# AI4quantum/twisteRL

Hardware: NVIDIA B200
Metric: rollout env-steps/sec incl. policy fwd (puzzle15 PPO) (higher is better)
Workload: dtype f16f8c (tcgen05; main products one-hot x table and h1 x W in fp16, their two correction products (table residue, activation residue) as fp8 MMAs, f32 accumulate; same 1e-3 bar as f16x2w16, tests/test_gpu_precision.py)

## Files before the change

### twisterl_b200/csrc/twr_forward_tc2.cu

```cuda
#include "twr_kernels.cuh"
#include "twr_tc_ptx.cuh"
#include "twr_step.cuh"

#include <atomic>
#include <cstdlib>
#include <cuda.h>
#include <cuda_fp16.h>
#include <cuda_fp8.h>
#include <map>
#include <mutex>

extern std::atomic<long long> g_twr_launches;

namespace {

constexpr int TM = 128;
constexpr int NTHREADS = 320;
constexpr int NEPI = 256;
constexpr int TILE_BYTES = 16384;
constexpr int NSLOTS = 8;
constexpr int MAX_KB1 = 4;
constexpr int MAX_OBS = 32;
constexpr int NCOPIES = 1;

constexpr int SM_A1 = 0;
constexpr int SM_RING = SM_A1 + MAX_KB1 * TILE_BYTES;
constexpr int SM_A8 = SM_RING;
constexpr int A8_TILES = 2;
constexpr int SM_MISC = SM_RING + NSLOTS * TILE_BYTES;
constexpr int SM_HEADW = SM_MISC;
constexpr int SM_B1 = SM_HEADW + 8192;
constexpr int SM_EMBB = SM_B1 + 1024;
constexpr int SM_PART = SM_EMBB + 4096;
constexpr int SM_PERM = SM_PART + 2 * TM * 8 * 4;
constexpr int SM_OPERM = SM_PERM + 4 * TM;
constexpr int OPERM_MAX = 2048;
constexpr int SM_BARS = SM_OPERM + OPERM_MAX;
constexpr int SM_TOTAL = SM_BARS + 512;
static_assert(SM_TOTAL <= 227 * 1024, "shared memory budget");

enum Bar { B_FULL0 = 0, B_EMPTY0 = NSLOTS, B_A1_FULL = 2 * NSLOTS, B_A1_EMPTY, B_D1_FULL0, B_D1_FULL1,
// ... 264 lines not shown
    float* headw = reinterpret_cast<float*>(smem + SM_HEADW);
    float* b1s = reinterpret_cast<float*>(smem + SM_B1);
    float* embb = reinterpret_cast<float*>(smem + SM_EMBB);
    float* part_s = reinterpret_cast<float*>(smem + SM_PART);
    int8_t* perm_s = reinterpret_cast<int8_t*>(smem + SM_PERM);
    uint8_t* operm_s = smem + SM_OPERM;
    const bool operm_smem = p.n_perms > 0 && p.obs_size <= 256 && p.n_perms * p.obs_size <= OPERM_MAX;
    const int NC = t.NC, NKB1 = t.NKB1;
    constexpr int H = HT;
    constexpr bool F8 = TERMS >= 16;
    static_assert(!F8 || TERMS == 19, "fp8 corrections replace exactly the terms of f16x2w16");
    constexpr int NS = F8 ? NSLOTS - A8_TILES : NSLOTS;
    constexpr int RING = F8 ? SM_RING + A8_TILES * TILE_BYTES : SM_RING;
    const int terms = TERMS >= 0 ? (TERMS & 7) : (a.tc_terms ? (a.tc_terms & 7) : 7);
    const bool g1_lo = (terms & 1) != 0, g2_alo = (terms & 2) != 0, g2_wlo = (terms & 4) != 0;
    const int NKB8 = t.NKB8;
    constexpr uint32_t idesc2 = H == 256 ? IDESC_256x256 : IDESC_256x128;
    constexpr int g2_units = H == 256 ? 4 : 2;

    if (threadIdx.x == 0) {
        for (int i = 0; i < NSLOTS; ++i) { mbar_init(bar(B_FULL0 + i), 1); mbar_init(bar(B_EMPTY0 + i), 1); }
        mbar_init(bar(B_A1_FULL), 2 * TM); mbar_init(bar(B_A1_EMPTY), 1);
        mbar_init(bar(B_D1_FULL0), 1); mbar_init(bar(B_D1_FULL1), 1);
        mbar_init(bar(B_A2_FULL0), 2 * NEPI); mbar_init(bar(B_A2_FULL1), 2 * NEPI);
        mbar_init(bar(B_D2_FULL), 1); mbar_init(bar(B_D2_EMPTY), 2 * NEPI);
        asm volatile("fence.mbarrier_init.release.cluster;" ::: "memory");
    }
    for (int i = threadIdx.x; i < (MAX_KB1 + (F8 ? A8_TILES : 0)) * TILE_BYTES / 16; i += NTHREADS)
        reinterpret_cast<uint4*>(smem + SM_A1)[i] = make_uint4(0, 0, 0, 0);
    for (int i = threadIdx.x; i < H; i += NTHREADS) {
        for (int o = 0; o < 4; ++o) headw[o * H + i] = o < p.A ? p.wa[(size_t)i * p.A + o] : 0.0f;
        headw[4 * H + i] = p.wv[i];
        b1s[i] = p.b1[i];
    }
    for (int i = threadIdx.x; i < t.E; i += NTHREADS) embb[i] = F8 ? p.emb_b[i] * H1_SCALE8 : p.emb_b[i];
    if (operm_smem)
        for (int i = threadIdx.x; i < p.n_perms * p.obs_size; i += NTHREADS) operm_s[i] = (uint8_t)p.obs_perms[i];
    uint8_t* aperm_s = smem + SM_BARS + 384;
    const bool aperm_smem = p.n_perms > 0 && p.n_perms * p.A <= 128;
    if (aperm_smem)
        for (int i = threadIdx.x; i < p.n_perms * p.A; i += NTHREADS) aperm_s[i] = (uint8_t)p.act_perms[i];
    if (warp == 1) {
        asm volatile("tcgen05.alloc.cta_group::2.sync.aligned.shared::cta.b32 [%0], %1;" ::"r"(smem_u32(tmem_slot)), "r"(512u));
        asm volatile("tcgen05.relinquish_alloc_permit.cta_group::2.sync.aligned;");
    }
    fence_async_smem();
    tc_fence_before();
    __syncthreads();
    cluster_sync();
    tc_fence_after();
    const uint32_t tmem = *tmem_slot;
    const uint32_t D2_COL = 0, D1_COL = 256;
    const bool timed = a.dbg != nullptr;
    long long* trace = (timed && blockIdx.x == 0) ? a.dbg + 148 * 16 : nullptr;
    auto stamp = [&](int item, int ev) { if (trace && item < 8) trace[item * 32 + ev] = clock64(); };

    if (warp == 0) {
        if (lane == 0) {
            const int img_row0 = t.row0 + ((pair_id % NCOPIES) * 2 + crank) * (int)slots_per_rank(t) * (TILE_BYTES / 128);
            const int g1_row0 = img_row0, g2_row0 = img_row0 + (int)slots_g1(t) * (TILE_BYTES / 128);
            uint32_t use = 0;
            long long w_empty = 0;
            auto push = [&](int row) {
                const uint32_t slot = use % NS, round = use / NS;
                mbar_wait_t(bar(B_EMPTY0 + slot), (round & 1u) ^ 1u, w_empty, timed);
                if (a.dbg_flags & 2) {
                    if (crank == 0) mbar_arrive(bar(B_FULL0 + slot));
                } else {
                    if (crank == 0) mbar_expect_tx(bar(B_FULL0 + slot), 2 * TILE_BYTES);
                    tma_load_2sm(sbase + RING + slot * TILE_BYTES, &tmap, 0, row, bar(B_FULL0 + slot));
                }
                ++use;
            };
            auto push_g1 = [&](int sc) {
                for (int i = 0; i < 2 * NKB1; ++i)
                    if (!(i & 1) || g1_lo) push(g1_row0 + (sc * 2 * NKB1 + i) * (TILE_BYTES / 128));
            };
            auto push_g2 = [&](int j) {
                for (int u = 0; u < g2_units; ++u)
                    if (!(u & 1) || g2_wlo) push(g2_row0 + (j * g2_units + u) * (TILE_BYTES / 128));
            };
            if constexpr (F8) {
                const int n1 = NKB1 + NKB8, n2 = 2 * (H == 256 ? 3 : 2);
                for (int it = 0; it < n_items; ++it)
                    for (int sc = 0; sc < NC / 2; ++sc) {
                        for (int u = 0; u < n1; ++u) push(g1_row0 + (sc * n1 + u) * (TILE_BYTES / 128));
                        for (int u = 0; u < n2; ++u) push(g2_row0 + (sc * n2 + u) * (TILE_BYTES / 128));
                    }
            } else {
                for (int it = 0; it < n_items; ++it)
                    for (int sc = 0; sc < NC / 2; ++sc) { push_g1(sc); push_g2(2 * sc); push_g2(2 * sc + 1); }
            }
            if (a.dbg) a.dbg[blockIdx.x * 16 + 8] = w_empty;
        }
        __syncwarp();
    } else if (warp == 1) {
        if (lane == 0 && crank == 0) {
            uint32_t use = 0, d1use = 0, a2use = 0;
            long long w_slot = 0, w_a1 = 0, w_a2 = 0, w_d2 = 0, w_slot_g1 = 0, w_slot_first = 0;
            const long long t_begin = clock64();
            auto wait_slot = [&]() -> uint32_t {
                const uint32_t slot = use % NS, round = use / NS;
                mbar_wait_cluster_t(bar(B_FULL0 + slot), round & 1u, w_slot, timed);
                tc_fence_after();
                ++use;
                return slot;
            };
            for (int it = 0; it < n_items; ++it) {
                mbar_wait_cluster_t(bar(B_A1_FULL), it & 1, w_a1, timed);
                tc_fence_after();
                stamp(it, 0);
                auto g1 = [&](int sc) {
                    stamp(it, 1 + 2 * sc);
                    const uint32_t d = tmem + D1_COL;
                    if constexpr (F8) {
                        constexpr uint32_t I8_256 = idesc8(256, 1, 0), I8_128 = idesc8(128, 1, 0);
                        const bool on = !(a.dbg_flags & 8);
                        for (int kb = 0; kb < NKB1 - 1; ++kb) {
                            const uint64_t ad = make_desc(sbase + SM_A1 + kb * TILE_BYTES);
// ... 158 lines not shown
                                const uint32_t sidx = H == 256 ? (uint32_t)((u >> 1) * 4 + ks) : (uint32_t)ks;
                                const uint32_t ah = a_base + 32u * (sidx >> 1) + 8u * (sidx & 1u);
                                const uint64_t bk = H == 256 ? bd + 2u * ks : bd + (uint64_t)((ks >> 2) * (8192 >> 4)) + 2u * (ks & 3);
                                tc2_mma_ts(d, ah, bk, idesc2, !(first && ks == 0));
                                if (part == 0 && g2_alo) tc2_mma_ts(d, ah + 16u, bk, idesc2, 1u);
                            }
                        }
                        tc2_commit(bar(B_EMPTY0 + slot));
                    }
                    ++a2use;
                    if (j == NC - 1) tc2_commit(bar(B_D2_FULL));
                };
                for (int sc = 0; sc < NC / 2; ++sc) { g1(sc); g2(2 * sc); g2(2 * sc + 1); }
                stamp(it, 9);
            }
            if (a.dbg) {
                long long* d = a.dbg + blockIdx.x * 16;
                d[0] = clock64() - t_begin; d[1] = w_slot; d[2] = w_a1; d[3] = w_a2; d[4] = w_d2; d[5] = my_tiles;
                d[6] = w_slot_g1; d[7] = w_slot_first;
            }
        }
        __syncwarp();
    } else {
        const int quarter = warp & 3;
        const int chalf = (warp - 2) >> 2;
        const int row = quarter * 32 + lane;
        const uint32_t lane_addr = ((uint32_t)(quarter * 32)) << 16;
        const int n_obs = p.n_obs;
        uint32_t d1use = 0;
        int perm_cur = -1, perm_next = -1;
        long long w_d1 = 0, w_d2f = 0, w_a1e = 0, c_epi1 = 0, c_build = 0, c_epi2 = 0;
        const long long t_begin = clock64();
        const uint32_t l_a1_full = lbar(B_A1_FULL), l_d2_empty = lbar(B_D2_EMPTY);
        const uint32_t l_a2_full0 = lbar(B_A2_FULL0), l_a2_full1 = lbar(B_A2_FULL1);
        float ba_r[4];
#pragma unroll
        for (int o = 0; o < 4; ++o) ba_r[o] = o < p.A ? p.ba[o] : 0.0f;
        const float bv_r = p.bv[0];

        struct Pre { int64_t pos; int64_t e; uint4 c; int step; };
        struct Ent { int group, step, extra; };
        Ent e_prev{0, 0, 0}, e_cur{0, 0, 0}, e_next{0, 0, 0};
        sched_item(sch, pair_id, 0, e_cur.group, e_cur.step, e_cur.extra);
        if (n_items > 1) sched_item(sch, pair_id, 1, e_next.group, e_next.step, e_next.extra);
        auto prefetch = [&](const Ent& en) -> Pre {
            const int group = en.group, step = en.step, extra = en.extra;
            if (extra == 1 && step == sch.sA0 && sch.sA0 > 0) wait_handoff(a.bal_flags + sch.gA, 2 * sch.sA0);
            Pre q; q.pos = ((int64_t)group * 2 + crank) * TM + row; q.e = 0; q.c = make_uint4(0, 0, 0, 0); q.step = step;
            if (q.pos < n) {
                q.e = a.live ? a.live[q.pos] : q.pos;
                if (!a.obs_rows) q.c = __ldcg(a.cells + q.e);
            }
            return q;
        };
        auto build_a1 = [&](int it, const Pre& q) -> int {
            const int64_t pos = q.pos;
            const int t_cur = a.t + q.step;
            int perm = -1;
            EnvState s; s.blank = 0; s.depth = 0;
            s.lo = (uint64_t)q.c.x | ((uint64_t)q.c.y << 32);
            s.hi = (uint64_t)q.c.z | ((uint64_t)q.c.w << 32);
            if (pos < n) {
                if (a.perm_idx) {
                    perm = a.perm_idx[pos];
                } else if (p.n_perms > 0 && a.t >= 0) {
                    uint32_t w[4];
                    philox4x32_10(a.ids.gid((uint32_t)q.e), (uint32_t)t_cur, TWR_RNG_PERM, a.cid, (uint32_t)a.seed,
                                  (uint32_t)(a.seed >> 32), w);
                    perm = (int)mulhi_u32(w[0], (uint32_t)p.n_perms);
                }
            }
            const uint32_t rx = (uint32_t)row & 7u;
            const uint32_t row_base = ((uint32_t)row >> 3) * 1024u + rx * 128u;
            const bool fast = a.env.kind == 0 && !a.obs_rows && (perm < 0 || operm_smem) && n_obs <= 16 && t.cN == 0;
            const uint8_t* otab = perm >= 0 ? operm_s + perm * p.obs_size : nullptr;
            if (threadIdx.x == 192) stamp(it, 20);
            mbar_wait_t(bar(B_A1_EMPTY), (it & 1) ^ 1, w_a1e, timed);
            if (threadIdx.x == 192) stamp(it, 21);
            for (int kb = 0; kb < NKB1; ++kb) {
                uint4* dst = reinterpret_cast<uint4*>(smem + SM_A1 + kb * TILE_BYTES + quarter * 4096) + lane;
#pragma unroll
                for (int j = 0; j < 8; ++j) dst[j * 32] = make_uint4(0, 0, 0, 0);
            }
            if constexpr (F8) {
                for (int kb = 0; kb < NKB8; ++kb) {
                    uint4* dst = reinterpret_cast<uint4*>(smem + SM_A8 + kb * TILE_BYTES + quarter * 4096) + lane;
#pragma unroll
                    for (int j = 0; j < 8; ++j) dst[j * 32] = make_uint4(0, 0, 0, 0);
                }
            }
            __syncwarp();
            auto set8 = [&](uint32_t r) {
                if constexpr (F8) {
                    const uint32_t k8 = r & 127u;
                    smem[SM_A8 + (r >> 7) * TILE_BYTES + row_base + ((((k8 >> 4) ^ rx) & 7u) << 4) + (k8 & 15u)] = ONE8;
                }
            };
            if (fast) {
#pragma unroll
                for (int i = 0; i < 16; ++i) {
                    if (i < n_obs) {
                        const uint32_t v = (uint32_t)(((i < 8) ? s.lo : s.hi) >> (8 * (i & 7))) & 0xFFu;
                        uint32_t r = pos < n ? (uint32_t)(i * a.env.N) + v : 0u;
                        if (otab && pos < n) r = otab[r];
                        const uint32_t k = r & 63u;
                        *reinterpret_cast<__half*>(smem + SM_A1 + (r >> 6) * TILE_BYTES + row_base + ((((k >> 3) ^ rx) & 7u) << 4) + (k & 7u) * 2u) =
                            __ushort_as_half(0x3C00);
                        set8(r);
                    }
                }
            } else {
                for (int i = 0; i < n_obs; ++i) {
                    uint32_t r = 0;
                    if (pos < n) {
                        r = a.obs_rows ? (uint32_t)a.obs_rows[pos * n_obs + i] : (uint32_t)(i * a.env.N) + env_board(a.env, s, i);
                        if (perm >= 0)
                            r = operm_smem ? (uint32_t)operm_s[perm * p.obs_size + (int)r] : (uint32_t)p.obs_perms[(size_t)perm * p.obs_size + r];
                        if (t.cN > 0) r = (r / (uint32_t)t.cN) * 4u + (r % (uint32_t)t.cN);
                    }
                    const uint32_t k = r & 63u;
                    *reinterpret_cast<__half*>(smem + SM_A1 + (r >> 6) * TILE_BYTES + row_base + ((((k >> 3) ^ rx) & 7u) << 4) + (k & 7u) * 2u) =
                        __ushort_as_half(0x3C00);
                    set8(r);
                }
            }
            perm_s[(it & 3) * TM + row] = (int8_t)perm;
            fence_async_smem();
            mbar_arrive_cluster(l_a1_full);
            if (threadIdx.x == 192) stamp(it, 22);
            return perm;
        };
        auto split2 = [g2_alo](float x0, float x1, uint32_t& hi, uint32_t& lo) {
            if (g2_alo) {
                asm("cvt.rz.relu.f16x2.f32 %0, %1, %2;" : "=r"(hi) : "f"(x1), "f"(x0));
                const float2 hf = __half22float2(*reinterpret_cast<const __half2*>(&hi));
                asm("cvt.rn.relu.f16x2.f32 %0, %1, %2;" : "=r"(lo) : "f"(x1 - hf.y), "f"(x0 - hf.x));
            } else {
                asm("cvt.rn.relu.f16x2.f32 %0, %1, %2;" : "=r"(hi) : "f"(x1), "f"(x0));
                lo = 0u;
            }
        };

        auto split4 = [](float x0, float x1, float x2, float x3, uint32_t& hi01, uint32_t& hi23, uint32_t& lo) {
            asm("cvt.rz.relu.f16x2.f32 %0, %1, %2;" : "=r"(hi01) : "f"(x1), "f"(x0));
            asm("cvt.rz.relu.f16x2.f32 %0, %1, %2;" : "=r"(hi23) : "f"(x3), "f"(x2));
            const float2 f01 = __half22float2(*reinterpret_cast<const __half2*>(&hi01)), f23 = __half22float2(*reinterpret_cast<const __half2*>(&hi23));
            const float2 r01 = __fadd2_rn(make_float2(x0, x1), make_float2(-f01.x, -f01.y));
            const float2 r23 = __fadd2_rn(make_float2(x2, x3), make_float2(-f23.x, -f23.y));
            uint16_t l01, l23;
            asm("cvt.rn.satfinite.relu.e5m2x2.f32 %0, %1, %2;" : "=h"(l01) : "f"(r01.y), "f"(r01.x));
            asm("cvt.rn.satfinite.relu.e5m2x2.f32 %0, %1, %2;" : "=h"(l23) : "f"(r23.y), "f"(r23.x));
            lo = (uint32_t)l01 | ((uint32_t)l23 << 16);
        };

        const bool build_early = my_tiles > 1 || t_count == 1;
        auto epi1 = [&](int it, int c) {
            const uint32_t buf = d1use & 1u;
            mbar_wait_t(bar(B_D1_FULL0 + buf), (d1use >> 1) & 1u, w_d1, timed);
            tc_fence_after();
            if (threadIdx.x == 64) stamp(it, 10 + c);
            const long long t_e1 = timed ? clock64() : 0;
            if (!(a.dbg_flags & 1)) {
                uint32_t v0[32], v1[32];
                const uint32_t taddr = tmem + lane_addr + D1_COL + buf * 128u + (uint32_t)chalf * 64u;
                tc_ld32(taddr, v0);
                tc_ld32(taddr + 32u, v1);
                tc_wait_ld();
                const float* bias = embb + c * 128 + chalf * 64;
                uint32_t w[32];
                if constexpr (F8) {
                    auto addb = [&](uint32_t v, const float& b) -> float {
                        if constexpr (FOLD) return __uint_as_float(v); else return __uint_as_float(v) + b;
                    };
#pragma unroll
                    for (int e4 = 0; e4 < 8; ++e4)
                        split4(addb(v0[4 * e4], bias[4 * e4]), addb(v0[4 * e4 + 1], bias[4 * e4 + 1]),
                               addb(v0[4 * e4 + 2], bias[4 * e4 + 2]), addb(v0[4 * e4 + 3], bias[4 * e4 + 3]),
                               w[2 * e4], w[2 * e4 + 1], w[16 + e4]);
#pragma unroll
                    for (int e4 = 24; e4 < 32; ++e4) w[e4] = 0u;
                    tc_st32(taddr, w);
#pragma unroll
                    for (int e4 = 0; e4 < 8; ++e4)
                        split4(addb(v1[4 * e4], bias[32 + 4 * e4]), addb(v1[4 * e4 + 1], bias[32 + 4 * e4 + 1]),
                               addb(v1[4 * e4 + 2], bias[32 + 4 * e4 + 2]), addb(v1[4 * e4 + 3], bias[32 + 4 * e4 + 3]),
                               w[2 * e4], w[2 * e4 + 1], w[16 + e4]);
                    tc_st32(taddr + 32u, w);
                } else {
#pragma unroll
                    for (int e2 = 0; e2 < 16; ++e2)
                        split2(__uint_as_float(v0[2 * e2]) + bias[2 * e2], __uint_as_float(v0[2 * e2 + 1]) + bias[2 * e2 + 1], w[e2], w[16 + e2]);
                    tc_st32(taddr, w);
#pragma unroll
                    for (int e2 = 0; e2 < 16; ++e2)
                        split2(__uint_as_float(v1[2 * e2]) + bias[32 + 2 * e2], __uint_as_float(v1[2 * e2 + 1]) + bias[32 + 2 * e2 + 1], w[e2], w[16 + e2]);
                    tc_st32(taddr + 32u, w);
                }
                tc_wait_st();
            }
            tc_fence_before();
            mbar_arrive_cluster(buf ? l_a2_full1 : l_a2_full0);
            if (timed) c_epi1 += clock64() - t_e1;
            if (threadIdx.x == 64) stamp(it, 14 + c);
            ++d1use;
        };
        struct Saved { float out[4]; float value; int perm; int64_t pos; int step, group, extra; bool valid; };
        auto run_step = [&](const Saved& v) {
            const bool active = v.pos < n;
            if (a.fused) {
                const int e = active ? (a.live ? a.live[v.pos] : (int)v.pos) : 0;
                StepArgs sa = a.step;
                sa.t = a.t + v.step;
                const bool alive = active && (t_count == 1 || a.cb.ep_len[e] == 0);
                collect_step_body(sa, a.cb, alive, e, make_float4(v.out[0], v.out[1], v.out[2], v.out[3]), v.value, v.perm,
                                  a.live_next);
            } else if (active) {
                a.logits[v.pos] = make_float4(v.out[0], v.out[1], v.out[2], v.out[3]);
                a.values[v.pos] = v.value;
            }
            if (v.extra) {
                asm volatile("bar.sync 4, %0;" ::"n"(NEPI / 2) : "memory");
                if (threadIdx.x == 64) { __threadfence(); atomicAdd(a.bal_flags + (v.group - sch.lanes * sch.P), 1); }
            }
        };
        const bool defer = build_early && a.fused && t_count > 1;
        Saved sv;
        sv.valid = false; sv.pos = 0; sv.step = 0; sv.group = 0; sv.extra = 0; sv.perm = -1; sv.value = 0.f;
        sv.out[0] = sv.out[1] = sv.out[2] = sv.out[3] = 0.f;

        if (chalf == 1) perm_next = build_a1(0, prefetch(e_cur));
        for (int it = 0; it < n_items; ++it) {
            Pre pre_next; pre_next.pos = 0; pre_next.e = 0; pre_next.c = make_uint4(0, 0, 0, 0); pre_next.step = 0;
            int c_done = 0;
            if (defer) {
                const bool dep = it >= 1 && it + 1 < n_items && e_prev.group == e_next.group;
                for (; c_done < 2 && c_done < NC; ++c_done) epi1(it, c_done);
                if (chalf == 1 && it + 1 < n_items && !dep) pre_next = prefetch(e_next);
                if (chalf == 0 && sv.valid) {
                    if (threadIdx.x == 64) stamp(it, 23);
                    run_step(sv);
                    if (threadIdx.x == 64) stamp(it, 24);
                    sv.valid = false;
                    if (dep) asm volatile("bar.arrive 3, %0;" ::"n"(NEPI) : "memory");
                }
                if (chalf == 1 && dep) {
                    asm volatile("bar.sync 3, %0;" ::"n"(NEPI) : "memory");
                    pre_next = prefetch(e_next);
                }
            } else if (build_early && chalf == 1 && it + 1 < n_items) {
                if (t_count > 1 && it >= 1) asm volatile("bar.sync 3, %0;" ::"n"(NEPI) : "memory");
                pre_next = prefetch(e_next);
            }
            for (; c_done < NC; ++c_done) epi1(it, c_done);
            {
                const long long t_b = timed ? clock64() : 0;
                if (build_early && chalf == 1 && it + 1 < n_items) perm_next = build_a1(it + 1, pre_next);
                if (timed) c_build += clock64() - t_b;
            }

            mbar_wait_t(bar(B_D2_FULL), it & 1, w_d2f, timed);
            tc_fence_after();
            if (threadIdx.x == 64) stamp(it, 18);
            const long long t_e2 = timed ? clock64() : 0;
            float2 acc2[5];
#pragma unroll
            for (int o = 0; o < 5; ++o) acc2[o] = make_float2(0.f, 0.f);
#pragma unroll 1
            for (int q = 0; q < H / 128; ++q) {
                uint32_t v0[32], v1[32];
                const uint32_t col0 = (uint32_t)(chalf * (H / 2)) + (uint32_t)q * 64u;
                tc_ld32(tmem + lane_addr + D2_COL + col0, v0);
                tc_ld32(tmem + lane_addr + D2_COL + col0 + 32u, v1);
                tc_wait_ld();
#pragma unroll
                for (int j4 = 0; j4 < 16; ++j4) {
                    const int col = (int)col0 + 4 * j4;
                    const float4 bb = *reinterpret_cast<const float4*>(b1s + col);
                    float hv[4];
#pragma unroll
                    for (int k = 0; k < 4; ++k) {
                        const int j = 4 * j4 + k;
                        hv[k] = __uint_as_float(j < 32 ? v0[j & 31] : v1[j & 31]);
                    }
                    float2 h01 = __fadd2_rn(make_float2(hv[0], hv[1]), make_float2(bb.x, bb.y));
                    float2 h23 = __fadd2_rn(make_float2(hv[2], hv[3]), make_float2(bb.z, bb.w));
                    h01.x = fmaxf(h01.x, 0.f); h01.y = fmaxf(h01.y, 0.f); h23.x = fmaxf(h23.x, 0.f); h23.y = fmaxf(h23.y, 0.f);
#pragma unroll
                    for (int o = 0; o < 5; ++o) {
                        const float4 w = *reinterpret_cast<const float4*>(headw + o * H + col);
                        acc2[o] = __ffma2_rn(h01, make_float2(w.x, w.y), acc2[o]);
                        acc2[o] = __ffma2_rn(h23, make_float2(w.z, w.w), acc2[o]);
                    }
                }
            }
            float acc[5];
#pragma unroll
            for (int o = 0; o < 5; ++o) acc[o] = acc2[o].x + acc2[o].y;
            tc_fence_before();
            mbar_arrive_cluster(l_d2_empty);
            float* ps = part_s + ((it & 1) * TM + row) * 8;
            if (chalf == 1) {
                *reinterpret_cast<float4*>(ps) = make_float4(acc[0], acc[1], acc[2], acc[3]);
                ps[4] = acc[4];
            }
            if (threadIdx.x == 64) stamp(it, 25);
            asm volatile("bar.sync 1, %0;" ::"n"(NEPI) : "memory");
            if (threadIdx.x == 64) stamp(it, 26);
            if (chalf == 0) {
                Saved cur;
                cur.group = e_cur.group; cur.step = e_cur.step; cur.extra = e_cur.extra;
                cur.pos = ((int64_t)cur.group * 2 + crank) * TM + row;
                cur.valid = true;
                cur.out[0] = cur.out[1] = cur.out[2] = cur.out[3] = 0.f;
                cur.value = 0.f;
                perm_cur = perm_s[(it & 3) * TM + row];
                cur.perm = perm_cur;
                if (cur.pos < n) {
                    const float4 o4 = *reinterpret_cast<const float4*>(ps);
                    acc[0] += o4.x; acc[1] += o4.y; acc[2] += o4.z; acc[3] += o4.w; acc[4] += ps[4];
                    float l[4];
#pragma unroll
                    for (int o = 0; o < 4; ++o) l[o] = o < p.A ? acc[o] + ba_r[o] : 0.0f;
#pragma unroll
                    for (int o = 0; o < 4; ++o) cur.out[o] = l[o];
                    if (perm_cur >= 0) {
#pragma unroll
                        for (int o = 0; o < 4; ++o) {
                            if (o < p.A) {
                                const int src = aperm_smem ? (int)aperm_s[perm_cur * p.A + o] : p.act_perms[perm_cur * p.A + o];
                                cur.out[o] = src == 0 ? l[0] : src == 1 ? l[1] : src == 2 ? l[2] : l[3];
                            }
                        }
                    }
                    cur.value = acc[4] + bv_r;
                }
                if (defer && it + 1 < n_items) {
                    sv = cur;
                } else {
                    run_step(cur);
                    if (!defer && build_early && t_count > 1 && it + 2 < n_items) asm volatile("bar.arrive 3, %0;" ::"n"(NEPI) : "memory");
                }
            }
            if (!build_early && it + 1 < n_items) {
                asm volatile("bar.sync 2, %0;" ::"n"(NEPI) : "memory");
                if (chalf == 1) perm_next = build_a1(it + 1, prefetch(e_next));
            }
            e_prev = e_cur; e_cur = e_next;
            if (it + 2 < n_items) sched_item(sch, pair_id, it + 2, e_next.group, e_next.step, e_next.extra);
            if (timed) c_epi2 += clock64() - t_e2;
            if (threadIdx.x == 64) stamp(it, 19);
        }
        if (a.dbg && threadIdx.x == 64) {
            long long* d = a.dbg + blockIdx.x * 16;
            d[9] = clock64() - t_begin; d[10] = w_d1; d[11] = w_d2f; d[12] = w_a1e; d[13] = c_epi1; d[14] = c_build; d[15] = c_epi2;
        }
    }

    tc_fence_before();
    __syncthreads();
    cluster_sync();
    if (warp == 1) {
        tc_fence_after();
        asm volatile("tcgen05.dealloc.cta_group::2.sync.aligned.b32 %0, %1;" ::"r"(tmem), "r"(512u));
    }
}

Tc2Params make_params2(const PolicyDev& p, bool f8 = false) {
    Tc2Params t;
    t.E = p.E; t.H = p.H; t.NC = p.E / 128; t.cN = p.tc_compact_n;
    t.NKB1 = ((p.tc_compact_n > 0 ? 4 * p.tc_compact_n : p.obs_size) + 63) / 64;
    t.NKB8 = (t.NKB1 + 1) / 2;
    t.f8 = 0; t.row0 = 0; t.fold = 0;
    if (f8) {
        t.row0 = (int)((size_t)NCOPIES * 2 * slots_per_rank(t) * (TILE_BYTES / 128));
        t.f8 = 1;
        t.fold = p.tc_fold;
    }
    return t;
}

struct DevState {
    int sms = 0;
    int max_clusters = -1;
    bool attr_set = false;
// ... 122 lines not shown
```

Baseline: 1.443 billion.

## Split epilogue warps into producer and consumer teams for warp specialization

Raises the block to 576 threads and splits the epilogue into two 256-thread teams. Team 0 builds the one-hot A1 tiles and runs the first-layer epilogue (split into fp16 plus fp8 residue). Team 1 consumes D2 and runs the head, run_step and env update. TMA and MMA move to warps 16 and 17, and the teams coordinate through named barriers indexed by item. The aim is to overlap the serial epi2/step work with the epi1/build work of the next item, at the cost of more registers, lower occupancy and more barrier traffic.

```diff
diff --git a/twisterl_b200/csrc/twr_forward_tc2.cu b/twisterl_b200/csrc/twr_forward_tc2.cu
--- a/twisterl_b200/csrc/twr_forward_tc2.cu
+++ b/twisterl_b200/csrc/twr_forward_tc2.cu
@@ -15,8 +15,10 @@
 namespace {
 
 constexpr int TM = 128;
-constexpr int NTHREADS = 320;
-constexpr int NEPI = 256;
+constexpr int NTHREADS = 576;
+constexpr int NTEAM = 256;
+constexpr int W_TMA = 16, W_MMA = 17;
+constexpr int T_CONS = 320;
 constexpr int TILE_BYTES = 16384;
 constexpr int NSLOTS = 8;
 constexpr int MAX_KB1 = 4;
@@ -327,8 +329,8 @@
         for (int i = 0; i < NSLOTS; ++i) { mbar_init(bar(B_FULL0 + i), 1); mbar_init(bar(B_EMPTY0 + i), 1); }
         mbar_init(bar(B_A1_FULL), 2 * TM); mbar_init(bar(B_A1_EMPTY), 1);
         mbar_init(bar(B_D1_FULL0), 1); mbar_init(bar(B_D1_FULL1), 1);
-        mbar_init(bar(B_A2_FULL0), 2 * NEPI); mbar_init(bar(B_A2_FULL1), 2 * NEPI);
-        mbar_init(bar(B_D2_FULL), 1); mbar_init(bar(B_D2_EMPTY), 2 * NEPI);
+        mbar_init(bar(B_A2_FULL0), 2 * NTEAM); mbar_init(bar(B_A2_FULL1), 2 * NTEAM);
+        mbar_init(bar(B_D2_FULL), 1); mbar_init(bar(B_D2_EMPTY), 2 * NTEAM);
         asm volatile("fence.mbarrier_init.release.cluster;" ::: "memory");
     }
     for (int i = threadIdx.x; i < (MAX_KB1 + (F8 ? A8_TILES : 0)) * TILE_BYTES / 16; i += NTHREADS)
@@ -345,7 +347,7 @@
     const bool aperm_smem = p.n_perms > 0 && p.n_perms * p.A <= 128;
     if (aperm_smem)
         for (int i = threadIdx.x; i < p.n_perms * p.A; i += NTHREADS) aperm_s[i] = (uint8_t)p.act_perms[i];
-    if (warp == 1) {
+    if (warp == W_MMA) {
         asm volatile("tcgen05.alloc.cta_group::2.sync.aligned.shared::cta.b32 [%0], %1;" ::"r"(smem_u32(tmem_slot)), "r"(512u));
         asm volatile("tcgen05.relinquish_alloc_permit.cta_group::2.sync.aligned;");
     }
@@ -360,7 +362,7 @@
     long long* trace = (timed && blockIdx.x == 0) ? a.dbg + 148 * 16 : nullptr;
     auto stamp = [&](int item, int ev) { if (trace && item < 8) trace[item * 32 + ev] = clock64(); };
 
-    if (warp == 0) {
+    if (warp == W_TMA) {
         if (lane == 0) {
             const int img_row0 = t.row0 + ((pair_id % NCOPIES) * 2 + crank) * (int)slots_per_rank(t) * (TILE_BYTES / 128);
             const int g1_row0 = img_row0, g2_row0 = img_row0 + (int)slots_g1(t) * (TILE_BYTES / 128);
@@ -399,7 +401,7 @@
             if (a.dbg) a.dbg[blockIdx.x * 16 + 8] = w_empty;
         }
         __syncwarp();
-    } else if (warp == 1) {
+    } else if (warp == W_MMA) {
         if (lane == 0 && crank == 0) {
             uint32_t use = 0, d1use = 0, a2use = 0;
             long long w_slot = 0, w_a1 = 0, w_a2 = 0, w_d2 = 0, w_slot_g1 = 0, w_slot_first = 0;
@@ -604,344 +606,318 @@
         }
         __syncwarp();
     } else {
+        const int team = warp >> 3;
         const int quarter = warp & 3;
-        const int chalf = (warp - 2) >> 2;
+        const int chalf = (warp >> 2) & 1;
         const int row = quarter * 32 + lane;
         const uint32_t lane_addr = ((uint32_t)(quarter * 32)) << 16;
-        const int n_obs = p.n_obs;
-        uint32_t d1use = 0;
-        int perm_cur = -1, perm_next = -1;
-        long long w_d1 = 0, w_d2f = 0, w_a1e = 0, c_epi1 = 0, c_build = 0, c_epi2 = 0;
-        const long long t_begin = clock64();
-        const uint32_t l_a1_full = lbar(B_A1_FULL), l_d2_empty = lbar(B_D2_EMPTY);
-        const uint32_t l_a2_full0 = lbar(B_A2_FULL0), l_a2_full1 = lbar(B_A2_FULL1);
-        float ba_r[4];
-#pragma unroll
-        for (int o = 0; o < 4; ++o) ba_r[o] = o < p.A ? p.ba[o] : 0.0f;
-        const float bv_r = p.bv[0];
-
-        struct Pre { int64_t pos; int64_t e; uint4 c; int step; };
-        struct Ent { int group, step, extra; };
-        Ent e_prev{0, 0, 0}, e_cur{0, 0, 0}, e_next{0, 0, 0};
-        sched_item(sch, pair_id, 0, e_cur.group, e_cur.step, e_cur.extra);
-        if (n_items > 1) sched_item(sch, pair_id, 1, e_next.group, e_next.step, e_next.extra);
-        auto prefetch = [&](const Ent& en) -> Pre {
-            const int group = en.group, step = en.step, extra = en.extra;
-            if (extra == 1 && step == sch.sA0 && sch.sA0 > 0) wait_handoff(a.bal_flags + sch.gA, 2 * sch.sA0);
-            Pre q; q.pos = ((int64_t)group * 2 + crank) * TM + row; q.e = 0; q.c = make_uint4(0, 0, 0, 0); q.step = step;
-            if (q.pos < n) {
-                q.e = a.live ? a.live[q.pos] : q.pos;
-                if (!a.obs_rows) q.c = __ldcg(a.cells + q.e);
-            }
-            return q;
-        };
-        auto build_a1 = [&](int it, const Pre& q) -> int {
-            const int64_t pos = q.pos;
-            const int t_cur = a.t + q.step;
-            int perm = -1;
-            EnvState s; s.blank = 0; s.depth = 0;
-            s.lo = (uint64_t)q.c.x | ((uint64_t)q.c.y << 32);
-            s.hi = (uint64_t)q.c.z | ((uint64_t)q.c.w << 32);
-            if (pos < n) {
-                if (a.perm_idx) {
-                    perm = a.perm_idx[pos];
-                } else if (p.n_perms > 0 && a.t >= 0) {
-                    uint32_t w[4];
-                    philox4x32_10(a.ids.gid((uint32_t)q.e), (uint32_t)t_cur, TWR_RNG_PERM, a.cid, (uint32_t)a.seed,
-                                  (uint32_t)(a.seed >> 32), w);
-                    perm = (int)mulhi_u32(w[0], (uint32_t)p.n_perms);
-                }
-            }
-            const uint32_t rx = (uint32_t)row & 7u;
-            const uint32_t row_base = ((uint32_t)row >> 3) * 1024u + rx * 128u;
-            const bool fast = a.env.kind == 0 && !a.obs_rows && (perm < 0 || operm_smem) && n_obs <= 16 && t.cN == 0;
-            const uint8_t* otab = perm >= 0 ? operm_s + perm * p.obs_size : nullptr;
-            if (threadIdx.x == 192) stamp(it, 20);
-            mbar_wait_t(bar(B_A1_EMPTY), (it & 1) ^ 1, w_a1e, timed);
-            if (threadIdx.x == 192) stamp(it, 21);
-            for (int kb = 0; kb < NKB1; ++kb) {
-                uint4* dst = reinterpret_cast<uint4*>(smem + SM_A1 + kb * TILE_BYTES + quarter * 4096) + lane;
-#pragma unroll
-                for (int j = 0; j < 8; ++j) dst[j * 32] = make_uint4(0, 0, 0, 0);
-            }
-            if constexpr (F8) {
-                for (int kb = 0; kb < NKB8; ++kb) {
-                    uint4* dst = reinterpret_cast<uint4*>(smem + SM_A8 + kb * TILE_BYTES + quarter * 4096) + lane;
+        const bool build_early = my_tiles > 1 || t_count == 1;
+        const bool sync3 = t_count > 1;
+        if (team == 0) {
+            const int n_obs = p.n_obs;
+            uint32_t d1use = 0;
+            long long w_d1 = 0, w_a1e = 0, c_epi1 = 0, c_build = 0;
+            struct Pre { int64_t pos; int64_t e; uint4 c; int step; };
+            auto prefetch = [&](int it) -> Pre {
+                int group, step, extra;
+                sched_item(sch, pair_id, it, group, step, extra);
+                if (extra == 1 && step == sch.sA0 && sch.sA0 > 0) wait_handoff(a.bal_flags + sch.gA, 2 * sch.sA0);
+                Pre q; q.pos = ((int64_t)group * 2 + crank) * TM + row; q.e = 0; q.c = make_uint4(0, 0, 0, 0); q.step = step;
+                if (q.pos < n) {
+                    q.e = a.live ? a.live[q.pos] : q.pos;
+                    if (!a.obs_rows) q.c = __ldcg(a.cells + q.e);
+                }
+                return q;
+            };
+            auto build_a1 = [&](int it, const Pre& q) {
+                const int64_t pos = q.pos;
+                const int t_cur = a.t + q.step;
+                int perm = -1;
+                EnvState s; s.blank = 0; s.depth = 0;
+                s.lo = (uint64_t)q.c.x | ((uint64_t)q.c.y << 32);
+                s.hi = (uint64_t)q.c.z | ((uint64_t)q.c.w << 32);
+                if (pos < n) {
+                    if (a.perm_idx) {
+                        perm = a.perm_idx[pos];
+                    } else if (p.n_perms > 0 && a.t >= 0) {
+                        uint32_t w[4];
+                        philox4x32_10(a.ids.gid((uint32_t)q.e), (uint32_t)t_cur, TWR_RNG_PERM, a.cid, (uint32_t)a.seed,
+                                      (uint32_t)(a.seed >> 32), w);
+                        perm = (int)mulhi_u32(w[0], (uint32_t)p.n_perms);
+                    }
+                }
+                const uint32_t rx = (uint32_t)row & 7u;
+                const uint32_t row_base = ((uint32_t)row >> 3) * 1024u + rx * 128u;
+                const bool fast = a.env.kind == 0 && !a.obs_rows && (perm < 0 || operm_smem) && n_obs <= 16 && t.cN == 0;
+                const uint8_t* otab = perm >= 0 ? operm_s + perm * p.obs_size : nullptr;
+                if (threadIdx.x == 192) stamp(it, 20);
+                mbar_wait_t(bar(B_A1_EMPTY), (it & 1) ^ 1, w_a1e, timed);
+                if (threadIdx.x == 192) stamp(it, 21);
+                for (int kb = 0; kb < NKB1; ++kb) {
+                    uint4* dst = reinterpret_cast<uint4*>(smem + SM_A1 + kb * TILE_BYTES + quarter * 4096) + lane;
 #pragma unroll
                     for (int j = 0; j < 8; ++j) dst[j * 32] = make_uint4(0, 0, 0, 0);
                 }
-            }
-            __syncwarp();
-            auto set8 = [&](uint32_t r) {
                 if constexpr (F8) {
-                    const uint32_t k8 = r & 127u;
-                    smem[SM_A8 + (r >> 7) * TILE_BYTES + row_base + ((((k8 >> 4) ^ rx) & 7u) << 4) + (k8 & 15u)] = ONE8;
-                }
-            };
-            if (fast) {
-#pragma unroll
-                for (int i = 0; i < 16; ++i) {
-                    if (i < n_obs) {
-                        const uint32_t v = (uint32_t)(((i < 8) ? s.lo : s.hi) >> (8 * (i & 7))) & 0xFFu;
-                        uint32_t r = pos < n ? (uint32_t)(i * a.env.N) + v : 0u;
-                        if (otab && pos < n) r = otab[r];
+                    for (int kb = 0; kb < NKB8; ++kb) {
+                        uint4* dst = reinterpret_cast<uint4*>(smem + SM_A8 + kb * TILE_BYTES + quarter * 4096) + lane;
+#pragma unroll
+                        for (int j = 0; j < 8; ++j) dst[j * 32] = make_uint4(0, 0, 0, 0);
+                    }
+                }
+                __syncwarp();
+                auto set8 = [&](uint32_t r) {
+                    if constexpr (F8) {
+                        const uint32_t k8 = r & 127u;
+                        smem[SM_A8 + (r >> 7) * TILE_BYTES + row_base + ((((k8 >> 4) ^ rx) & 7u) << 4) + (k8 & 15u)] = ONE8;
+                    }
+                };
+                if (fast) {
+#pragma unroll
+                    for (int i = 0; i < 16; ++i) {
+                        if (i < n_obs) {
+                            const uint32_t v = (uint32_t)(((i < 8) ? s.lo : s.hi) >> (8 * (i & 7))) & 0xFFu;
+                            uint32_t r = pos < n ? (uint32_t)(i * a.env.N) + v : 0u;
+                            if (otab && pos < n) r = otab[r];
+                            const uint32_t k = r & 63u;
+                            *reinterpret_cast<__half*>(smem + SM_A1 + (r >> 6) * TILE_BYTES + row_base + ((((k >> 3) ^ rx) & 7u) << 4) + (k & 7u) * 2u) =
+                                __ushort_as_half(0x3C00);
+                            set8(r);
+                        }
+                    }
+                } else {
+                    for (int i = 0; i < n_obs; ++i) {
+                        uint32_t r = 0;
+                        if (pos < n) {
+                            r = a.obs_rows ? (uint32_t)a.obs_rows[pos * n_obs + i] : (uint32_t)(i * a.env.N) + env_board(a.env, s, i);
+                            if (perm >= 0)
+                                r = operm_smem ? (uint32_t)operm_s[perm * p.obs_size + (int)r] : (uint32_t)p.obs_perms[(size_t)perm * p.obs_size + r];
+                            if (t.cN > 0) r = (r / (uint32_t)t.cN) * 4u + (r % (uint32_t)t.cN);
+                        }
                         const uint32_t k = r & 63u;
                         *reinterpret_cast<__half*>(smem + SM_A1 + (r >> 6) * TILE_BYTES + row_base + ((((k >> 3) ^ rx) & 7u) << 4) + (k & 7u) * 2u) =
                             __ushort_as_half(0x3C00);
                         set8(r);
                     }
                 }
-            } else {
-                for (int i = 0; i < n_obs; ++i) {
-                    uint32_t r = 0;
-                    if (pos < n) {
-                        r = a.obs_rows ? (uint32_t)a.obs_rows[pos * n_obs + i] : (uint32_t)(i * a.env.N) + env_board(a.env, s, i);
-                        if (perm >= 0)
-                            r = operm_smem ? (uint32_t)operm_s[perm * p.obs_size + (int)r] : (uint32_t)p.obs_perms[(size_t)perm * p.obs_size + r];
-                        if (t.cN > 0) r = (r / (uint32_t)t.cN) * 4u + (r % (uint32_t)t.cN);
-                    }
-                    const uint32_t k = r & 63u;
-                    *reinterpret_cast<__half*>(smem + SM_A1 + (r >> 6) * TILE_BYTES + row_base + ((((k >> 3) ^ rx) & 7u) << 4) + (k & 7u) * 2u) =
-                        __ushort_as_half(0x3C00);
-                    set8(r);
+                perm_s[(it & 3) * TM + row] = (int8_t)perm;
+                asm volatile("bar.arrive %0, %1;" ::"r"(5 + (it & 3)), "n"(NTEAM) : "memory");
+                fence_async_smem();
+                mbar_arrive_cluster(lbar(B_A1_FULL));
+                if (threadIdx.x == 192) stamp(it, 22);
+            };
+            auto split2 = [g2_alo](float x0, float x1, uint32_t& hi, uint32_t& lo) {
+                if (g2_alo) {
+                    asm("cvt.rz.relu.f16x2.f32 %0, %1, %2;" : "=r"(hi) : "f"(x1), "f"(x0));
+                    const float2 hf = __half22float2(*reinterpret_cast<const __half2*>(&hi));
+                    asm("cvt.rn.relu.f16x2.f32 %0, %1, %2;" : "=r"(lo) : "f"(x1 - hf.y), "f"(x0 - hf.x));
+                } else {
+                    asm("cvt.rn.relu.f16x2.f32 %0, %1, %2;" : "=r"(hi) : "f"(x1), "f"(x0));
+                    lo = 0u;
+                }
+            };
+            auto split4 = [](float x0, float x1, float x2, float x3, uint32_t& hi01, uint32_t& hi23, uint32_t& lo) {
+                asm("cvt.rz.relu.f16x2.f32 %0, %1, %2;" : "=r"(hi01) : "f"(x1), "f"(x0));
+                asm("cvt.rz.relu.f16x2.f32 %0, %1, %2;" : "=r"(hi23) : "f"(x3), "f"(x2));
+                const float2 f01 = __half22float2(*reinterpret_cast<const __half2*>(&hi01)), f23 = __half22float2(*reinterpret_cast<const __half2*>(&hi23));
+                const float2 r01 = __fadd2_rn(make_float2(x0, x1), make_float2(-f01.x, -f01.y));
+                const float2 r23 = __fadd2_rn(make_float2(x2, x3), make_float2(-f23.x, -f23.y));
+                uint16_t l01, l23;
+                asm("cvt.rn.satfinite.relu.e5m2x2.f32 %0, %1, %2;" : "=h"(l01) : "f"(r01.y), "f"(r01.x));
+                asm("cvt.rn.satfinite.relu.e5m2x2.f32 %0, %1, %2;" : "=h"(l23) : "f"(r23.y), "f"(r23.x));
+                lo = (uint32_t)l01 | ((uint32_t)l23 << 16);
+            };
+            auto epi1 = [&](int it, int c) {
+                const uint32_t buf = d1use & 1u;
+                mbar_wait_t(bar(B_D1_FULL0 + buf), (d1use >> 1) & 1u, w_d1, timed);
+                tc_fence_after();
+                if (threadIdx.x == 64) stamp(it, 10 + c);
+                const long long t_e1 = timed ? clock64() : 0;
+                if (!(a.dbg_flags & 1)) {
+                    const uint32_t taddr0 = tmem + lane_addr + D1_COL + buf * 128u + (uint32_t)chalf * 64u;
+#pragma unroll
+                    for (int hh = 0; hh < 2; ++hh) {
+                        uint32_t v[32], w[32];
+                        const uint32_t taddr = taddr0 + 32u * hh;
+                        tc_ld32(taddr, v);
+                        tc_wait_ld();
+                        const float* bias = embb + c * 128 + chalf * 64 + 32 * hh;
+                        if constexpr (F8) {
+                            auto addb = [&](uint32_t x, const float& b) -> float {
+                                if constexpr (FOLD) return __uint_as_float(x); else return __uint_as_float(x) + b;
+                            };
+#pragma unroll
+                            for (int e4 = 0; e4 < 8; ++e4)
+                                split4(addb(v[4 * e4], bias[4 * e4]), addb(v[4 * e4 + 1], bias[4 * e4 + 1]),
+                                       addb(v[4 * e4 + 2], bias[4 * e4 + 2]), addb(v[4 * e4 + 3], bias[4 * e4 + 3]),
+                                       w[2 * e4], w[2 * e4 + 1], w[16 + e4]);
+#pragma unroll
+                            for (int e4 = 24; e4 < 32; ++e4) w[e4] = 0u;
+                        } else {
+#pragma unroll
+                            for (int e2 = 0; e2 < 16; ++e2)
+                                split2(__uint_as_float(v[2 * e2]) + bias[2 * e2], __uint_as_float(v[2 * e2 + 1]) + bias[2 * e2 + 1], w[e2], w[16 + e2]);
+                        }
+                        tc_st32(taddr, w);
+                    }
+                    tc_wait_st();
+                }
+                tc_fence_before();
+                mbar_arrive_cluster(buf ? lbar(B_A2_FULL1) : lbar(B_A2_FULL0));
+                if (timed) c_epi1 += clock64() - t_e1;
+                if (threadIdx.x == 64) stamp(it, 14 + c);
+                ++d1use;
+            };
+
+            const int c_pre = (build_early && NC >= 4) ? NC - 2 : NC;
+            if (chalf == 1) build_a1(0, prefetch(0));
+            for (int it = 0; it < n_items; ++it) {
+                const bool next = chalf == 1 && it + 1 < n_items;
+                Pre pre; pre.pos = 0; pre.e = 0; pre.c = make_uint4(0, 0, 0, 0); pre.step = 0;
+                auto fetch_next = [&]() {
+                    if (sync3 && (it >= 1 || !build_early)) asm volatile("bar.sync 3, %0;" ::"n"(NTEAM) : "memory");
+                    pre = prefetch(it + 1);
+                };
+                for (int c = 0; c < NC; ++c) {
+                    if (c == c_pre && next) fetch_next();
+                    epi1(it, c);
+                }
+                if (next) {
+                    const long long t_b = timed ? clock64() : 0;
+                    if (c_pre == NC) fetch_next();
+                    build_a1(it + 1, pre);
+                    if (timed) c_build += clock64() - t_b;
                 }
             }
-            perm_s[(it & 3) * TM + row] = (int8_t)perm;
-            fence_async_smem();
-            mbar_arrive_cluster(l_a1_full);
-            if (threadIdx.x == 192) stamp(it, 22);
-            return perm;
-        };
-        auto split2 = [g2_alo](float x0, float x1, uint32_t& hi, uint32_t& lo) {
-            if (g2_alo) {
-                asm("cvt.rz.relu.f16x2.f32 %0, %1, %2;" : "=r"(hi) : "f"(x1), "f"(x0));
-                const float2 hf = __half22float2(*reinterpret_cast<const __half2*>(&hi));
-                asm("cvt.rn.relu.f16x2.f32 %0, %1, %2;" : "=r"(lo) : "f"(x1 - hf.y), "f"(x0 - hf.x));
-            } else {
-                asm("cvt.rn.relu.f16x2.f32 %0, %1, %2;" : "=r"(hi) : "f"(x1), "f"(x0));
-                lo = 0u;
+            if (a.dbg && threadIdx.x == 64) { long long* d = a.dbg + blockIdx.x * 16; d[10] = w_d1; d[13] = c_epi1; }
+            if (a.dbg && threadIdx.x == 192) { long long* d = a.dbg + blockIdx.x * 16; d[12] = w_a1e; d[14] = c_build; }
+        } else {
+            long long w_d2f = 0, c_epi2 = 0;
+            float ba_r[4];
+#pragma unroll
+            for (int o = 0; o < 4; ++o) ba_r[o] = o < p.A ? p.ba[o] : 0.0f;
+            const float bv_r = p.bv[0];
+            if (a.dbg && threadIdx.x == T_CONS) a.dbg[blockIdx.x * 16 + 9] = clock64();
+            struct Saved { float out[4]; float value; int perm; int64_t pos; int step, group, extra; };
+            auto run_step = [&](const Saved& v) {
+                const bool active = v.pos < n;
+                if (a.fused) {
+                    const int e = active ? (a.live ? a.live[v.pos] : (int)v.pos) : 0;
+                    StepArgs sa = a.step;
+                    sa.t = a.t + v.step;
+                    const bool alive = active && (t_count == 1 || a.cb.ep_len[e] == 0);
+                    collect_step_body(sa, a.cb, alive, e, make_float4(v.out[0], v.out[1], v.out[2], v.out[3]), v.value, v.perm,
+                                      a.live_next);
+                } else if (active) {
+                    a.logits[v.pos] = make_float4(v.out[0], v.out[1], v.out[2], v.out[3]);
+                    a.values[v.pos] = v.value;
+                }
+                if (v.extra) {
+                    asm volatile("bar.sync 4, %0;" ::"n"(NTEAM / 2) : "memory");
+                    if (threadIdx.x == T_CONS) { __threadfence(); atomicAdd(a.bal_flags + (v.group - sch.lanes * sch.P), 1); }
+                }
+            };
+            for (int it = 0; it < n_items; ++it) {
+                mbar_wait_t(bar(B_D2_FULL), it & 1, w_d2f, timed);
+                tc_fence_after();
+                if (threadIdx.x == T_CONS) stamp(it, 18);
+                const long long t_e2 = timed ? clock64() : 0;
+                int perm_cur = -1;
+                if (chalf == 0) {
+                    asm volatile("bar.sync %0, %1;" ::"r"(5 + (it & 3)), "n"(NTEAM) : "memory");
+                    perm_cur = perm_s[(it & 3) * TM + row];
+                }
+                float2 acc2[5];
+#pragma unroll
+                for (int o = 0; o < 5; ++o) acc2[o] = make_float2(0.f, 0.f);
+#pragma unroll 1
+                for (int q = 0; q < H / 128; ++q) {
+                    uint32_t v0[32], v1[32];
+                    const uint32_t col0 = (uint32_t)(chalf * (H / 2)) + (uint32_t)q * 64u;
+                    tc_ld32(tmem + lane_addr + D2_COL + col0, v0);
+                    tc_ld32(tmem + lane_addr + D2_COL + col0 + 32u, v1);
+                    tc_wait_ld();
+                    if (q == H / 128 - 1) {
+                        tc_fence_before();
+                        mbar_arrive_cluster(lbar(B_D2_EMPTY));
+                    }
+#pragma unroll
+                    for (int j4 = 0; j4 < 16; ++j4) {
+                        const int col = (int)col0 + 4 * j4;
+                        const float4 bb = *reinterpret_cast<const float4*>(b1s + col);
+                        float hv[4];
+#pragma unroll
+                        for (int k = 0; k < 4; ++k) {
+                            const int j = 4 * j4 + k;
+                            hv[k] = __uint_as_float(j < 32 ? v0[j & 31] : v1[j & 31]);
+                        }
+                        float2 h01 = __fadd2_rn(make_float2(hv[0], hv[1]), make_float2(bb.x, bb.y));
+                        float2 h23 = __fadd2_rn(make_float2(hv[2], hv[3]), make_float2(bb.z, bb.w));
+                        h01.x = fmaxf(h01.x, 0.f); h01.y = fmaxf(h01.y, 0.f); h23.x = fmaxf(h23.x, 0.f); h23.y = fmaxf(h23.y, 0.f);
+#pragma unroll
+                        for (int o = 0; o < 5; ++o) {
+                            const float4 w = *reinterpret_cast<const float4*>(headw + o * H + col);
+                            acc2[o] = __ffma2_rn(h01, make_float2(w.x, w.y), acc2[o]);
+                            acc2[o] = __ffma2_rn(h23, make_float2(w.z, w.w), acc2[o]);
+                        }
+                    }
+                }
+                float acc[5];
+#pragma unroll
+                for (int o = 0; o < 5; ++o) acc[o] = acc2[o].x + acc2[o].y;
+                float* ps = part_s + ((it & 1) * TM + row) * 8;
+                if (chalf == 1) {
+                    *reinterpret_cast<float4*>(ps) = make_float4(acc[0], acc[1], acc[2], acc[3]);
+                    ps[4] = acc[4];
+                }
+                if (threadIdx.x == T_CONS) stamp(it, 25);
+                asm volatile("bar.sync 1, %0;" ::"n"(NTEAM) : "memory");
+                if (threadIdx.x == T_CONS) stamp(it, 26);
+                if (chalf == 0) {
+                    Saved cur;
+                    sched_item(sch, pair_id, it, cur.group, cur.step, cur.extra);
+                    cur.pos = ((int64_t)cur.group * 2 + crank) * TM + row;
+                    cur.out[0] = cur.out[1] = cur.out[2] = cur.out[3] = 0.f;
+                    cur.value = 0.f;
+                    cur.perm = perm_cur;
+                    if (cur.pos < n) {
+                        const float4 o4 = *reinterpret_cast<const float4*>(ps);
+                        acc[0] += o4.x; acc[1] += o4.y; acc[2] += o4.z; acc[3] += o4.w; acc[4] += ps[4];
+                        float l[4];
+#pragma unroll
+                        for (int o = 0; o < 4; ++o) l[o] = o < p.A ? acc[o] + ba_r[o] : 0.0f;
+#pragma unroll
+                        for (int o = 0; o < 4; ++o) cur.out[o] = l[o];
+                        if (perm_cur >= 0) {
+#pragma unroll
+                            for (int o = 0; o < 4; ++o) {
+                                if (o < p.A) {
+                                    const int src = aperm_smem ? (int)aperm_s[perm_cur * p.A + o] : p.act_perms[perm_cur * p.A + o];
+                                    cur.out[o] = src == 0 ? l[0] : src == 1 ? l[1] : src == 2 ? l[2] : l[3];
+                                }
+                            }
+                        }
+                        cur.value = acc[4] + bv_r;
+                    }
+                    if (threadIdx.x == T_CONS) stamp(it + 1, 23);
+                    run_step(cur);
+                    if (threadIdx.x == T_CONS) stamp(it + 1, 24);
+                    if (sync3 && it + (build_early ? 2 : 1) < n_items) asm volatile("bar.sync 3, %0;" ::"n"(NTEAM) : "memory");
+                }
+                if (timed) c_epi2 += clock64() - t_e2;
+                if (threadIdx.x == T_CONS) stamp(it, 19);
             }
-        };
-
-        auto split4 = [](float x0, float x1, float x2, float x3, uint32_t& hi01, uint32_t& hi23, uint32_t& lo) {
-            asm("cvt.rz.relu.f16x2.f32 %0, %1, %2;" : "=r"(hi01) : "f"(x1), "f"(x0));
-            asm("cvt.rz.relu.f16x2.f32 %0, %1, %2;" : "=r"(hi23) : "f"(x3), "f"(x2));
-            const float2 f01 = __half22float2(*reinterpret_cast<const __half2*>(&hi01)), f23 = __half22float2(*reinterpret_cast<const __half2*>(&hi23));
-            const float2 r01 = __fadd2_rn(make_float2(x0, x1), make_float2(-f01.x, -f01.y));
-            const float2 r23 = __fadd2_rn(make_float2(x2, x3), make_float2(-f23.x, -f23.y));
-            uint16_t l01, l23;
-            asm("cvt.rn.satfinite.relu.e5m2x2.f32 %0, %1, %2;" : "=h"(l01) : "f"(r01.y), "f"(r01.x));
-            asm("cvt.rn.satfinite.relu.e5m2x2.f32 %0, %1, %2;" : "=h"(l23) : "f"(r23.y), "f"(r23.x));
-            lo = (uint32_t)l01 | ((uint32_t)l23 << 16);
-        };
-
-        const bool build_early = my_tiles > 1 || t_count == 1;
-        auto epi1 = [&](int it, int c) {
-            const uint32_t buf = d1use & 1u;
-            mbar_wait_t(bar(B_D1_FULL0 + buf), (d1use >> 1) & 1u, w_d1, timed);
-            tc_fence_after();
-            if (threadIdx.x == 64) stamp(it, 10 + c);
-            const long long t_e1 = timed ? clock64() : 0;
-            if (!(a.dbg_flags & 1)) {
-                uint32_t v0[32], v1[32];
-                const uint32_t taddr = tmem + lane_addr + D1_COL + buf * 128u + (uint32_t)chalf * 64u;
-                tc_ld32(taddr, v0);
-                tc_ld32(taddr + 32u, v1);
-                tc_wait_ld();
-                const float* bias = embb + c * 128 + chalf * 64;
-                uint32_t w[32];
-                if constexpr (F8) {
-                    auto addb = [&](uint32_t v, const float& b) -> float {
-                        if constexpr (FOLD) return __uint_as_float(v); else return __uint_as_float(v) + b;
-                    };
-#pragma unroll
-                    for (int e4 = 0; e4 < 8; ++e4)
-                        split4(addb(v0[4 * e4], bias[4 * e4]), addb(v0[4 * e4 + 1], bias[4 * e4 + 1]),
-                               addb(v0[4 * e4 + 2], bias[4 * e4 + 2]), addb(v0[4 * e4 + 3], bias[4 * e4 + 3]),
-                               w[2 * e4], w[2 * e4 + 1], w[16 + e4]);
-#pragma unroll
-                    for (int e4 = 24; e4 < 32; ++e4) w[e4] = 0u;
-                    tc_st32(taddr, w);
-#pragma unroll
-                    for (int e4 = 0; e4 < 8; ++e4)
-                        split4(addb(v1[4 * e4], bias[32 + 4 * e4]), addb(v1[4 * e4 + 1], bias[32 + 4 * e4 + 1]),
-                               addb(v1[4 * e4 + 2], bias[32 + 4 * e4 + 2]), addb(v1[4 * e4 + 3], bias[32 + 4 * e4 + 3]),
-                               w[2 * e4], w[2 * e4 + 1], w[16 + e4]);
-                    tc_st32(taddr + 32u, w);
-                } else {
-#pragma unroll
-                    for (int e2 = 0; e2 < 16; ++e2)
-                        split2(__uint_as_float(v0[2 * e2]) + bias[2 * e2], __uint_as_float(v0[2 * e2 + 1]) + bias[2 * e2 + 1], w[e2], w[16 + e2]);
-                    tc_st32(taddr, w);
-#pragma unroll
-                    for (int e2 = 0; e2 < 16; ++e2)
-                        split2(__uint_as_float(v1[2 * e2]) + bias[32 + 2 * e2], __uint_as_float(v1[2 * e2 + 1]) + bias[32 + 2 * e2 + 1], w[e2], w[16 + e2]);
-                    tc_st32(taddr + 32u, w);
-                }
-                tc_wait_st();
+            if (a.dbg && threadIdx.x == T_CONS) {
+                long long* d = a.dbg + blockIdx.x * 16;
+                d[9] = clock64() - d[9]; d[11] = w_d2f; d[15] = c_epi2;
             }
-            tc_fence_before();
-            mbar_arrive_cluster(buf ? l_a2_full1 : l_a2_full0);
-            if (timed) c_epi1 += clock64() - t_e1;
-            if (threadIdx.x == 64) stamp(it, 14 + c);
-            ++d1use;
-        };
-        struct Saved { float out[4]; float value; int perm; int64_t pos; int step, group, extra; bool valid; };
-        auto run_step = [&](const Saved& v) {
-            const bool active = v.pos < n;
-            if (a.fused) {
-                const int e = active ? (a.live ? a.live[v.pos] : (int)v.pos) : 0;
-                StepArgs sa = a.step;
-                sa.t = a.t + v.step;
-                const bool alive = active && (t_count == 1 || a.cb.ep_len[e] == 0);
-                collect_step_body(sa, a.cb, alive, e, make_float4(v.out[0], v.out[1], v.out[2], v.out[3]), v.value, v.perm,
-                                  a.live_next);
-            } else if (active) {
-                a.logits[v.pos] = make_float4(v.out[0], v.out[1], v.out[2], v.out[3]);
-                a.values[v.pos] = v.value;
-            }
-            if (v.extra) {
-                asm volatile("bar.sync 4, %0;" ::"n"(NEPI / 2) : "memory");
-                if (threadIdx.x == 64) { __threadfence(); atomicAdd(a.bal_flags + (v.group - sch.lanes * sch.P), 1); }
-            }
-        };
-        const bool defer = build_early && a.fused && t_count > 1;
-        Saved sv;
-        sv.valid = false; sv.pos = 0; sv.step = 0; sv.group = 0; sv.extra = 0; sv.perm = -1; sv.value = 0.f;
-        sv.out[0] = sv.out[1] = sv.out[2] = sv.out[3] = 0.f;
-
-        if (chalf == 1) perm_next = build_a1(0, prefetch(e_cur));
-        for (int it = 0; it < n_items; ++it) {
-            Pre pre_next; pre_next.pos = 0; pre_next.e = 0; pre_next.c = make_uint4(0, 0, 0, 0); pre_next.step = 0;
-            int c_done = 0;
-            if (defer) {
-                const bool dep = it >= 1 && it + 1 < n_items && e_prev.group == e_next.group;
-                for (; c_done < 2 && c_done < NC; ++c_done) epi1(it, c_done);
-                if (chalf == 1 && it + 1 < n_items && !dep) pre_next = prefetch(e_next);
-                if (chalf == 0 && sv.valid) {
-                    if (threadIdx.x == 64) stamp(it, 23);
-                    run_step(sv);
-                    if (threadIdx.x == 64) stamp(it, 24);
-                    sv.valid = false;
-                    if (dep) asm volatile("bar.arrive 3, %0;" ::"n"(NEPI) : "memory");
-                }
-                if (chalf == 1 && dep) {
-                    asm volatile("bar.sync 3, %0;" ::"n"(NEPI) : "memory");
-                    pre_next = prefetch(e_next);
-                }
-            } else if (build_early && chalf == 1 && it + 1 < n_items) {
-                if (t_count > 1 && it >= 1) asm volatile("bar.sync 3, %0;" ::"n"(NEPI) : "memory");
-                pre_next = prefetch(e_next);
-            }
-            for (; c_done < NC; ++c_done) epi1(it, c_done);
-            {
-                const long long t_b = timed ? clock64() : 0;
-                if (build_early && chalf == 1 && it + 1 < n_items) perm_next = build_a1(it + 1, pre_next);
-                if (timed) c_build += clock64() - t_b;
-            }
-
-            mbar_wait_t(bar(B_D2_FULL), it & 1, w_d2f, timed);
-            tc_fence_after();
-            if (threadIdx.x == 64) stamp(it, 18);
-            const long long t_e2 = timed ? clock64() : 0;
-            float2 acc2[5];
-#pragma unroll
-            for (int o = 0; o < 5; ++o) acc2[o] = make_float2(0.f, 0.f);
-#pragma unroll 1
-            for (int q = 0; q < H / 128; ++q) {
-                uint32_t v0[32], v1[32];
-                const uint32_t col0 = (uint32_t)(chalf * (H / 2)) + (uint32_t)q * 64u;
-                tc_ld32(tmem + lane_addr + D2_COL + col0, v0);
-                tc_ld32(tmem + lane_addr + D2_COL + col0 + 32u, v1);
-                tc_wait_ld();
-#pragma unroll
-                for (int j4 = 0; j4 < 16; ++j4) {
-                    const int col = (int)col0 + 4 * j4;
-                    const float4 bb = *reinterpret_cast<const float4*>(b1s + col);
-                    float hv[4];
-#pragma unroll
-                    for (int k = 0; k < 4; ++k) {
-                        const int j = 4 * j4 + k;
-                        hv[k] = __uint_as_float(j < 32 ? v0[j & 31] : v1[j & 31]);
-                    }
-                    float2 h01 = __fadd2_rn(make_float2(hv[0], hv[1]), make_float2(bb.x, bb.y));
-                    float2 h23 = __fadd2_rn(make_float2(hv[2], hv[3]), make_float2(bb.z, bb.w));
-                    h01.x = fmaxf(h01.x, 0.f); h01.y = fmaxf(h01.y, 0.f); h23.x = fmaxf(h23.x, 0.f); h23.y = fmaxf(h23.y, 0.f);
-#pragma unroll
-                    for (int o = 0; o < 5; ++o) {
-                        const float4 w = *reinterpret_cast<const float4*>(headw + o * H + col);
-                        acc2[o] = __ffma2_rn(h01, make_float2(w.x, w.y), acc2[o]);
-                        acc2[o] = __ffma2_rn(h23, make_float2(w.z, w.w), acc2[o]);
-                    }
-                }
-            }
-            float acc[5];
-#pragma unroll
-            for (int o = 0; o < 5; ++o) acc[o] = acc2[o].x + acc2[o].y;
-            tc_fence_before();
-            mbar_arrive_cluster(l_d2_empty);
-            float* ps = part_s + ((it & 1) * TM + row) * 8;
-            if (chalf == 1) {
-                *reinterpret_cast<float4*>(ps) = make_float4(acc[0], acc[1], acc[2], acc[3]);
-                ps[4] = acc[4];
-            }
-            if (threadIdx.x == 64) stamp(it, 25);
-            asm volatile("bar.sync 1, %0;" ::"n"(NEPI) : "memory");
-            if (threadIdx.x == 64) stamp(it, 26);
-            if (chalf == 0) {
-                Saved cur;
-                cur.group = e_cur.group; cur.step = e_cur.step; cur.extra = e_cur.extra;
-                cur.pos = ((int64_t)cur.group * 2 + crank) * TM + row;
-                cur.valid = true;
-                cur.out[0] = cur.out[1] = cur.out[2] = cur.out[3] = 0.f;
-                cur.value = 0.f;
-                perm_cur = perm_s[(it & 3) * TM + row];
-                cur.perm = perm_cur;
-                if (cur.pos < n) {
-                    const float4 o4 = *reinterpret_cast<const float4*>(ps);
-                    acc[0] += o4.x; acc[1] += o4.y; acc[2] += o4.z; acc[3] += o4.w; acc[4] += ps[4];
-                    float l[4];
-#pragma unroll
-                    for (int o = 0; o < 4; ++o) l[o] = o < p.A ? acc[o] + ba_r[o] : 0.0f;
-#pragma unroll
-                    for (int o = 0; o < 4; ++o) cur.out[o] = l[o];
-                    if (perm_cur >= 0) {
-#pragma unroll
-                        for (int o = 0; o < 4; ++o) {
-                            if (o < p.A) {
-                                const int src = aperm_smem ? (int)aperm_s[perm_cur * p.A + o] : p.act_perms[perm_cur * p.A + o];
-                                cur.out[o] = src == 0 ? l[0] : src == 1 ? l[1] : src == 2 ? l[2] : l[3];
-                            }
-                        }
-                    }
-                    cur.value = acc[4] + bv_r;
-                }
-                if (defer && it + 1 < n_items) {
-                    sv = cur;
-                } else {
-                    run_step(cur);
-                    if (!defer && build_early && t_count > 1 && it + 2 < n_items) asm volatile("bar.arrive 3, %0;" ::"n"(NEPI) : "memory");
-                }
-            }
-            if (!build_early && it + 1 < n_items) {
-                asm volatile("bar.sync 2, %0;" ::"n"(NEPI) : "memory");
-                if (chalf == 1) perm_next = build_a1(it + 1, prefetch(e_next));
-            }
-            e_prev = e_cur; e_cur = e_next;
-            if (it + 2 < n_items) sched_item(sch, pair_id, it + 2, e_next.group, e_next.step, e_next.extra);
-            if (timed) c_epi2 += clock64() - t_e2;
-            if (threadIdx.x == 64) stamp(it, 19);
-        }
-        if (a.dbg && threadIdx.x == 64) {
-            long long* d = a.dbg + blockIdx.x * 16;
-            d[9] = clock64() - t_begin; d[10] = w_d1; d[11] = w_d2f; d[12] = w_a1e; d[13] = c_epi1; d[14] = c_build; d[15] = c_epi2;
         }
     }
 
     tc_fence_before();
     __syncthreads();
     cluster_sync();
-    if (warp == 1) {
+    if (warp == W_MMA) {
         tc_fence_after();
         asm volatile("tcgen05.dealloc.cta_group::2.sync.aligned.b32 %0, %1;" ::"r"(tmem), "r"(512u));
     }
```

Result: slower. 1.423 billion, median of 6 (-1.4%).
